# iric-soft/km

Hardware: AMD Instinct MI355X
Metric: find_mutation_targets_per_sec (higher is better)
Workload: dtype u64

## Files before the change

### km_amd/csrc/walk_kernel.h

```cpp
#pragma once
#include "device_common.h"

namespace kmd {

constexpr uint32_t ST_NODE = 1, ST_ONSTACK = 2, ST_POPPED = 3;
__device__ inline uint16_t slot_meta(uint32_t state, uint32_t idx) { return (uint16_t)((state << 14) | (idx & 0x3FFFu)); }
__device__ inline uint32_t meta_state(uint16_t m) { return (uint32_t)m >> 14; }
__device__ inline uint32_t meta_index(uint16_t m) { return (uint32_t)m & 0x3FFFu; }
constexpr uint32_t T_OK = 0, T_NODE_LIMIT = 1, T_REPEAT = 2, T_EMPTY = 3, T_BAD_BASE = 4,
                   T_INTERNAL = 5, T_NEEDS_BIG = 100;
constexpr uint64_t DFS_STEP_LIMIT = 1ull << 32;
constexpr uint32_t SEED_BLOCK = 256;

constexpr uint32_t POOL_GROUPS = 64;
constexpr uint32_t POOL_CTR_STRIDE = 16;
constexpr uint32_t NOT_BARE = 0xFFFFFFFFu;

struct EpiArgs {
  unsigned long long* counters;
  uint64_t path_pool, run_pool;
  uint32_t* p_target;
  uint64_t* p_runbase;
  uint32_t* p_nruns;
  uint32_t* p_len;
  uint32_t* p_mincov;
  uint32_t* r_start;
  uint32_t* r_len;
  uint32_t* g_status;
  uint32_t* t_npaths;
  uint32_t* t_pathbase;
  uint32_t* t_nruns;
  uint32_t* t_refmax;
  uint32_t* left;
  uint32_t* n_left;
  uint32_t* t_eremoved;
  uint32_t* t_enonref;
};
constexpr uint32_t EPI_CHUNKS = 3;
constexpr uint32_t EPI_MAX_BUBBLES = 8;

struct __attribute__((aligned(16))) BranchFrame {
  uint4 c4;
  uint32_t depth, mask, brk, pad;
};

struct WalkArgs {
  TableView tab;
  const uint8_t* bases;
  const uint64_t* toff;
  uint64_t* packed;
  const uint64_t* woff;
  uint32_t n_targets;
  double ratio;
  int64_t n_cutoff;
  double nc;
  uint64_t thr_below;
  uint32_t thr_T;
  uint32_t max_stack, max_break, max_node;
  uint64_t* items;
  const uint32_t* item_off;
  uint32_t n_items;
  uint32_t* flagbits;
  const uint64_t* fw_off;
  uint32_t* tflag;
  uint32_t* flagged;
  uint32_t* n_flagged;
  uint4* flag_rec;
  uint32_t fast_extra;
  const EpiArgs* epi;
  const uint32_t* list;
  const uint32_t* n_list_dev;
  uint32_t n_list_host;
  uint64_t* node_kmer;
  uint32_t* node_cnt;
  uint64_t* node_base;
  uint32_t* node_cap;
  const uint64_t* node_base0;
  uint32_t* big_ctl;
  uint32_t* big_walk;
  uint32_t big_slots;
  uint32_t big_entry;
  uint64_t big_region;
  uint32_t big_prep;
  uint32_t* loop_list;
  uint32_t* loop_ctl;
  uint32_t loop_cap;
  uint32_t* t_eremoved;
  uint32_t* t_enonref;
  uint32_t* n_nodes;
  uint32_t* n_ref;
  uint32_t* status;
  unsigned long long* probes;
  unsigned long long* dfs_probes;
  unsigned long long* fetches;
  uint32_t hs_cap;
  uint32_t pcap;
  uint32_t words_cap;
  uint32_t fcap;
  uint32_t bcap;
  uint32_t dbg;
  uint32_t spec;
  unsigned char* g_ws;
  uint64_t g_stride;
  unsigned char* f_ws;
  uint64_t f_stride;
  unsigned long long* stamps;
  unsigned long long* pool_counters;
};

__host__ __device__ inline uint64_t walk_frame_bytes(uint32_t fcap) {
  return (((uint64_t)fcap * 16) + 15) & ~15ull;
}
__host__ __device__ inline uint64_t walk_lds_bytes(uint32_t hs_cap, uint32_t words_cap, uint32_t bcap, uint32_t pcap,
                                                   uint32_t pos_elt) {
  uint64_t b = 0;
  b += (uint64_t)hs_cap * 8;
  b += (uint64_t)words_cap * 8;
  b += (uint64_t)bcap * 32;
  b += (uint64_t)hs_cap * 2;
  b += (uint64_t)pcap * pos_elt;
  return (b + 15) & ~15ull;
}
__host__ __device__ inline uint64_t walk_ws_bytes(uint32_t hs_cap, uint32_t words_cap,
                                                  uint32_t fcap, uint32_t bcap, uint32_t pcap) {
  return walk_lds_bytes(hs_cap, words_cap, bcap, pcap, 4) + walk_frame_bytes(fcap);
}

__device__ inline uint32_t set_home(uint64_t key, uint32_t cap) {
  uint32_t h = (uint32_t)key ^ ((uint32_t)(key >> 32) * 0x85EBCA6Bu);
  h *= 0x9E3779B1u;
  h ^= h >> 15;
  return __umulhi(h, cap);
}

template <int SH = 0>
__device__ inline int set_insert_lane(uint64_t* keys, uint32_t cap, uint64_t key, bool* was_new) {
  uint32_t s = set_home(key >> SH, cap);
  for (uint32_t step = 0; step < cap; ++step) {
    unsigned long long old = atomicCAS(reinterpret_cast<unsigned long long*>(&keys[s]),
                                       (unsigned long long)EMPTY, (unsigned long long)key);
    if (old == EMPTY) { *was_new = true; return (int)s; }
    if (old == key) { *was_new = false; return (int)s; }
    if (++s == cap) s = 0;
  }
  *was_new = false;
  return -1;
}

template <int SH = 0>
__device__ inline int set_lookup_lane(const uint64_t* keys, uint32_t cap, uint64_t key, bool* found) {
  uint32_t s = set_home(key >> SH, cap);
  for (uint32_t step = 0; step < cap; ++step) {
    const uint64_t kv = keys[s];
    if (kv == key) { *found = true; return (int)s; }
    if (kv == EMPTY) { *found = false; return (int)s; }
    if (++s == cap) s = 0;
  }
  *found = false;
  return -1;
}

template <int SH = 0>
__device__ inline int set_find(const uint64_t* keys, uint32_t cap, uint64_t key, bool* found) {
  const uint32_t lane = (uint32_t)lane_id();
  uint32_t base = set_home(key >> SH, cap);
  for (uint32_t scanned = 0; scanned < cap + 64; scanned += 64) {
    uint32_t s = base + lane;
    if (s >= cap) s -= cap;
    const uint64_t kv = keys[s];
    const unsigned long long mm = __ballot(kv == key);
    const unsigned long long me = __ballot(kv == EMPTY);
    if (mm | me) {
      const int lm = mm ? (__ffsll((long long)mm) - 1) : 64;
      const int le = me ? (__ffsll((long long)me) - 1) : 64;
      uint32_t pos = base + (uint32_t)(lm < le ? lm : le);
      if (pos >= cap) pos -= cap;
      *found = lm < le;
      return (int)pos;
    }
    base += 64;
    if (base >= cap) base -= cap;
  }
  *found = false;
  return -1;
}

constexpr uint32_t PACK_WAVES = 4;
__global__ __launch_bounds__(64 * PACK_WAVES) void k_pack(WalkArgs a) {
  constexpr uint32_t PACK_LDS_WORDS = 192;
  __shared__ uint64_t lds_words[PACK_WAVES][PACK_LDS_WORDS];
  uint64_t* const mine = lds_words[threadIdx.x >> 6];
  const uint32_t t = blockIdx.x * PACK_WAVES + (threadIdx.x >> 6);
  const uint32_t lane = (uint32_t)lane_id();
  if (t >= a.n_targets) return;
  const uint64_t off = a.toff[t];
  const uint64_t L = a.toff[t + 1] - off;
  const uint64_t wo = a.woff[t];
  const uint64_t fwo = a.fw_off[t];
  const uint64_t nbase = a.node_base0[t];
  const uint64_t item0 = a.item_off[t];
  const uint32_t nwords = (uint32_t)((L + 31) >> 5);
  const uint32_t n_ref = (L >= (uint64_t)a.tab.k) ? (uint32_t)(L - a.tab.k + 1) : 0;
  uint32_t bad = 0;
  for (uint32_t c = 0; c * 8 <= nwords; ++c) {
    const uint64_t p = (uint64_t)c * 256 + lane * 4;
    uint32_t byte = 0;
    uint32_t four = 0;
    if (p + 4 <= L) {
      __builtin_memcpy(&four, a.bases + off + p, 4);
    } else {
#pragma unroll
      for (uint32_t j = 0; j < 4; ++j)
        if (p + j < L) four |= (uint32_t)a.bases[off + p + j] << (8 * j);
    }
#pragma unroll
    for (uint32_t j = 0; j < 4; ++j) {
      uint32_t code = 0;
      if (p + j < L) {
        const uint32_t ch = (four >> (8 * j)) & 0xDFu;
        bad |= (ch != 'A' && ch != 'C' && ch != 'G' && ch != 'T') ? 1u : 0u;
        code = ((ch >> 1) ^ (ch >> 2)) & 3u;
      }
      byte = (byte << 2) | code;
    }
    uint64_t v = (uint64_t)byte << (56 - 8 * (lane & 7));
    v |= __shfl_xor(v, 1);
    v |= __shfl_xor(v, 2);
    v |= __shfl_xor(v, 4);
    const uint32_t w = c * 8 + (lane >> 3);
    if ((lane & 7) == 0 && w <= nwords) {
      a.packed[wo + w] = v;
      if (w < PACK_LDS_WORDS) mine[w] = v;
    }
  }
  const bool in_lds = nwords < PACK_LDS_WORDS;
  for (uint32_t w = lane; w < (n_ref + 31) / 32; w += 64) a.flagbits[fwo + w] = 0;
  const int any_bad = __any((int)bad);
  uint32_t st = T_OK;
  if (n_ref == 0) st = T_EMPTY;
  else if (any_bad) st = T_BAD_BASE;
  else if (a.max_stack > 0 && n_ref > a.max_node) st = T_NODE_LIMIT;
  if (in_lds) {
    asm volatile("s_waitcnt lgkmcnt(0)" ::: "memory");
  } else {
    __builtin_amdgcn_fence(__ATOMIC_RELEASE, "wavefront");
    asm volatile("s_waitcnt vmcnt(0)" ::: "memory");
    __builtin_amdgcn_fence(__ATOMIC_ACQUIRE, "wavefront");
  }
  {
    const uint32_t n_it = (n_ref + SEED_BLOCK - 1) / SEED_BLOCK;
    uint64_t* rec0 = a.items + 16ull * item0;
    for (uint32_t x = lane; x < n_it * 16; x += 64) {
      const uint32_t q = x >> 4, f = x & 15;
      uint64_t v;
      if (f == 0) v = (uint64_t)t | ((uint64_t)(q * SEED_BLOCK) << 32);
      else if (f == 1) v = (uint64_t)n_ref | ((uint64_t)(st == T_OK ? 1u : 0u) << 32);
      else if (f == 2) v = nbase;
      else if (f == 3) v = fwo | (wo << 32);
      else {
        const uint32_t w = q * (SEED_BLOCK / 32) + (f - 4);
        v = (w <= nwords) ? (in_lds ? mine[w] : a.packed[wo + w]) : 0ull;
      }
      rec0[x] = v;
    }
  }
  if (lane == 0) {
    a.status[t] = st;
    a.n_ref[t] = n_ref;
    a.n_nodes[t] = (st == T_OK || st == T_NODE_LIMIT) ? n_ref : 0;
    a.probes[t] = 0;
    a.dfs_probes[t] = 0;
    a.fetches[t] = 0;
    a.tflag[t] = 0;
    a.node_base[t] = nbase;
    a.node_cap[t] = n_ref + a.fast_extra;
    a.t_eremoved[t] = 0;
    a.t_enonref[t] = 0;
    if (t == 0) a.loop_ctl[0] = 0;
    if (t == 0 && a.big_ctl) { a.big_ctl[0] = 0; a.big_ctl[1] = 0; }
    if (t == 0) { a.n_flagged[0] = 0; a.n_flagged[1] = 0; a.n_flagged[2] = 0; }
  }
  {
    constexpr uint32_t CTR_PAIRS = (POOL_GROUPS * POOL_CTR_STRIDE + 16) / 2;
    ulonglong2* ctr = reinterpret_cast<ulonglong2*>(a.pool_counters);
    for (uint64_t i = (uint64_t)t * 64 + lane; i < CTR_PAIRS; i += (uint64_t)a.n_targets * 64)
      ctr[i] = make_ulonglong2(0ull, 0ull);
  }
}

#define KM_SEED_STAMP(n)                                                                  \
  do {                                                                                    \
    if constexpr (STAMPS) {                                                               \
      unsigned long long t_;                                                              \
      asm volatile("s_waitcnt vmcnt(0) lgkmcnt(0)\n\ts_memtime %0\n\ts_waitcnt lgkmcnt(0)" \
                   : "=s"(t_)::"memory");                                                 \
      ts[n] = t_;                                                                         \
    }                                                                                     \
  } while (0)

template <bool STAMPS, int K, bool FETCHES>
__global__ __launch_bounds__(SEED_BLOCK) void k_seed(WalkArgs a) {
  static_assert(SEED_BLOCK == 256, "the item record holds 12 words = 256 seeds + k - 1 + 1 bases");
  constexpr uint32_t RAW = SEED_BLOCK + 32;
  __shared__ uint32_t raw[RAW];
  unsigned long long ts[8] = {0, 0, 0, 0, 0, 0, 0, 0};
  unsigned long long real0 = 0;
  uint32_t probes_first = 0;
  if constexpr (STAMPS) real0 = __builtin_amdgcn_s_memrealtime();
  KM_SEED_STAMP(0);
  const TableView tab = specialized_view<K>(a.tab);
  const int k = tab.k;
  const uint32_t tid = threadIdx.x;
  const uint32_t lane = tid & 63u;
  const uint32_t W = (uint32_t)tab.w;
  const uint64_t* rec = a.items + 16ull * blockIdx.x;
  KM_SEED_STAMP(1);
  auto bits_at = [&](uint32_t q) -> uint64_t {
    const uint32_t w = q >> 5, sh = (q & 31) * 2;
    const uint64_t hi = rec[4 + w], lo = rec[5 + w];
    return (hi << sh) | ((lo >> 1) >> (63 - sh));
  };
  const uint64_t x = bits_at(tid);
  KM_SEED_STAMP(2);

  raw[tid] = mmer_scan_key(tab, x, tid);
  if (tid < W) raw[SEED_BLOCK + tid] = mmer_scan_key(tab, bits_at(SEED_BLOCK + tid), SEED_BLOCK + tid);
  const uint64_t h0 = rec[0], h1 = rec[1];
  const uint64_t nb = rec[2], fwo = rec[3] & 0xFFFFFFFFull;
  const uint32_t wo32 = (uint32_t)(rec[3] >> 32);
  if ((uint32_t)(h1 >> 32) == 0u) return;
  const uint32_t t = (uint32_t)h0;
  const uint32_t n_ref = (uint32_t)h1;
  const uint32_t i = (uint32_t)(h0 >> 32) + tid;
  __syncthreads();
  uint32_t m_rest;
  uint32_t m_last;
  if (W == 16) {
    const uint32_t* r = raw + tid + 1;
    const uint32_t m0 = min(min(r[0], r[1]), r[2]), m1 = min(min(r[3], r[4]), r[5]);
    const uint32_t m2 = min(min(r[6], r[7]), r[8]), m3 = min(min(r[9], r[10]), r[11]);
    const uint32_t m4 = min(min(r[12], r[13]), r[14]);
    m_rest = min(min(min(m0, m1), m2), min(m3, m4));
    m_last = r[15];
  } else {
    m_rest = ~0u;
    for (uint32_t j = 1; j < W; ++j) m_rest = min(m_rest, raw[tid + j]);
    m_last = raw[tid + W];
  }
  const uint32_t u_child = (min(m_rest, m_last) & SEL_POS) - (tid + 1);
  KM_SEED_STAMP(3);

  const uint64_t X = x >> (64 - 2 * k);
  const Key g = key_from_window(tab, X & tab.pmask, u_child);
  const DirPair dw = *reinterpret_cast<const DirPair*>(tab.dir + g.bucket);
  const bool head = i == 0;
  Key gq = g;
  DirPair dq = dw;
  if (head) {
    const uint32_t u_first = min(raw[0], m_rest) & SEL_POS;
    gq = key_from_window(tab, X >> 2, u_first);
    dq = *reinterpret_cast<const DirPair*>(tab.dir + gq.bucket);
  }
  KM_SEED_STAMP(4);
  const uint32_t S = (uint32_t)bucket_slots(dw.lo, dw.hi);
  const Slot* base = tab.slots + 2ull * dw.lo;
  const uint32_t pos = (uint32_t)home_slot(tab, g, S);
  const Slot* b0 = (S ? base : tab.slots) + pos;
  const uint4 first = *reinterpret_cast<const uint4*>(b0);
  const uint4 second = *reinterpret_cast<const uint4*>(b0 + 1);
  uint32_t Sq = 0, posq = 0;
  const Slot* baseq = tab.slots;
  uint4 firstq = first, secondq = second;
  if (head) {
    Sq = (uint32_t)bucket_slots(dq.lo, dq.hi);
    baseq = tab.slots + 2ull * dq.lo;
    posq = (uint32_t)home_slot(tab, gq, Sq);
    const Slot* bq = (Sq ? baseq : tab.slots) + posq;
    firstq = *reinterpret_cast<const uint4*>(bq);
    secondq = *reinterpret_cast<const uint4*>(bq + 1);
  }
  KM_SEED_STAMP(5);

  uint32_t fetch_l = 0;
  bool valid = false, triv = false, triv_child = false;
  if (i < n_ref) {
    valid = true;
    uint4 c4 = make_uint4(0, 0, 0, 0);
    if (S) c4 = bucket_resolve2(tab, g, base, S, pos, first, second, &fetch_l);
    c4 = finish_children(tab, X, g.flip, c4);
    KM_SEED_STAMP(6);
    if constexpr (STAMPS) probes_first = fetch_l;
    uint32_t nextb = 4;
    if (i + 1 < n_ref) {
      if (k < 32) {
        nextb = (uint32_t)(x >> (62 - 2 * k)) & 3u;
      } else {
        const uint32_t p = tid + (uint32_t)k;
        nextb = (uint32_t)(rec[4 + (p >> 5)] >> (62 - 2 * (p & 31))) & 3u;
      }
      a.node_cnt[nb + i + 1] = pick4(c4, nextb);
    }
    if (head) {
      uint4 cq = make_uint4(0, 0, 0, 0);
      if (Sq) cq = bucket_resolve2(tab, gq, baseq, Sq, posq, firstq, secondq, &fetch_l);
      const uint32_t sb = (uint32_t)(X & 3);
      uint32_t v = pick4(cq, gq.flip ? 3 - sb : sb);
      if (v == COUNT_ESCAPE) v = overflow_count(tab, X);
      a.node_cnt[nb] = v;
    }
    if (a.max_stack > 0) {
      const uint32_t mask = child_mask(c4, a.ratio, a.nc);
      triv = (mask == 0) || (nextb < 4 && mask == (1u << nextb));
      triv_child = triv && mask != 0;
      if (!triv) {
        atomicOr(&a.flagbits[fwo + (i >> 5)], 1u << (i & 31));
        if (atomicExch(&a.tflag[t], 1u) == 0u) {
          const uint32_t at = atomicAdd(a.n_flagged, 1u);
          a.flagged[at] = t;
          a.flag_rec[2 * at] = make_uint4(t, n_ref, (uint32_t)nb, (uint32_t)(nb >> 32));
          a.flag_rec[2 * at + 1] = make_uint4((uint32_t)fwo, wo32, 0u, 0u);
        }
      }
    }
  }
  const unsigned long long probes_w = (unsigned long long)__popcll(__ballot(valid)) +
                                      4ull * __popcll(__ballot(triv)) + __popcll(__ballot(triv_child));
  unsigned long long fetch_w = 0;
  if constexpr (FETCHES || STAMPS) {
    fetch_w = (unsigned long long)__popcll(__ballot(fetch_l >= 1)) + __popcll(__ballot(fetch_l >= 2));
    if (__any(fetch_l > 2)) {
      uint32_t extra = fetch_l > 2 ? fetch_l - 2 : 0;
      for (int o = 32; o > 0; o >>= 1) extra += __shfl_xor(extra, o);
      fetch_w += extra;
    }
  }
  if (lane == 0 && probes_w) {
    atomicAdd(&a.probes[t], probes_w);
    if constexpr (FETCHES || STAMPS) atomicAdd(&a.fetches[t], fetch_w);
  }
  if constexpr (STAMPS) {
    KM_SEED_STAMP(7);
    const unsigned long long real1 = __builtin_amdgcn_s_memrealtime();
    uint32_t pmax = probes_first, psum = probes_first;
    for (int o2 = 32; o2 > 0; o2 >>= 1) {
      const uint32_t v = __shfl_xor(pmax, o2);
      pmax = v > pmax ? v : pmax;
      psum += __shfl_xor(psum, o2);
    }
    if (lane == 0) {
      unsigned long long* o = a.stamps + 16ull * (blockIdx.x * (SEED_BLOCK / 64) + (tid >> 6));
      for (int q = 0; q < 8; ++q) o[q] = ts[q];
      o[8] = real0; o[9] = real1;
      o[10] = __builtin_amdgcn_s_getreg((31 << 11) | 4);
      o[11] = __builtin_amdgcn_s_getreg((31 << 11) | 20);
      o[12] = pmax; o[13] = psum;
    }
  }
}

constexpr uint32_t SEED_WAVE_KEYS = 96;
constexpr int SEED_WAVE_RUNS = 4;
constexpr uint32_t SEED_WAVE_LDS = SEED_WAVE_RUNS * SEED_WAVE_KEYS * 4;
template <int K, bool FETCHES, int NS>
__device__ __forceinline__ void seed_body(const WalkArgs a, const uint32_t item, const uint32_t wave) {
  static_assert(SEED_BLOCK == 256, "the item record holds 12 words = 256 seeds + k - 1 + 1 bases");
  static_assert(NS == 1 || NS == 2 || NS == 4, "one, two or all four runs of 64 seeds per wave");
  constexpr uint32_t WAVES = 4 / NS;
  extern __shared__ __align__(16) unsigned char smem[];
  uint32_t* const raw_all = reinterpret_cast<uint32_t*>(smem);
  const TableView tab = specialized_view<K>(a.tab);
  const int k = tab.k;
  const uint32_t lane = (uint32_t)lane_id();
  const uint32_t W = (uint32_t)tab.w;
  const uint64_t* rec = a.items + 16ull * item;
  auto bits_at = [&](uint32_t q) -> uint64_t {
    const uint32_t w = q >> 5, sh = (q & 31) * 2;
    const uint64_t hi = rec[4 + w], lo = rec[5 + w];
    return (hi << sh) | ((lo >> 1) >> (63 - sh));
  };
  struct Run {
    uint32_t tid, m_rest, u_child, S, pos;
    uint64_t x, X;
    Key g;
    DirPair dw;
    const Slot* base;
    uint4 first, second;
  };
  Run r0, r1, r2, r3;
  auto hash_keys = [&](Run& r, const uint32_t j) {
    r.tid = 64u * (wave + WAVES * j) + lane;
    r.x = bits_at(r.tid);
    uint32_t* raw = raw_all + SEED_WAVE_KEYS * j;
    raw[lane] = mmer_scan_key(tab, r.x, r.tid);
    if (lane < W) raw[64 + lane] = mmer_scan_key(tab, bits_at(r.tid + 64), r.tid + 64);
  };
  hash_keys(r0, 0);
  if constexpr (NS >= 2) hash_keys(r1, 1);
  if constexpr (NS == 4) { hash_keys(r2, 2); hash_keys(r3, 3); }
  const uint64_t h0 = rec[0], h1 = rec[1];
  const uint64_t nb = rec[2], fwo = rec[3] & 0xFFFFFFFFull;
  const uint32_t wo32 = (uint32_t)(rec[3] >> 32);
  if ((uint32_t)(h1 >> 32) == 0u) return;
  const uint32_t t = (uint32_t)h0;
  const uint32_t n_ref = (uint32_t)h1;
  const uint32_t i_first = (uint32_t)(h0 >> 32);
  if (i_first + 64u * wave >= n_ref) return;
  asm volatile("s_waitcnt lgkmcnt(0)" ::: "memory");
  auto minimizer = [&](Run& r, const uint32_t j) {
    const uint32_t* w = raw_all + SEED_WAVE_KEYS * j + lane + 1;
    uint32_t m_last;
    if (W == 16) {
      const uint32_t m0 = min(min(w[0], w[1]), w[2]), m1 = min(min(w[3], w[4]), w[5]);
      const uint32_t m2 = min(min(w[6], w[7]), w[8]), m3 = min(min(w[9], w[10]), w[11]);
      const uint32_t m4 = min(min(w[12], w[13]), w[14]);
      r.m_rest = min(min(min(m0, m1), m2), min(m3, m4));
      m_last = w[15];
    } else {
      r.m_rest = ~0u;
      for (uint32_t q = 1; q < W; ++q) r.m_rest = min(r.m_rest, w[q - 1]);
      m_last = w[W - 1];
    }
    r.u_child = (min(r.m_rest, m_last) & SEL_POS) - (r.tid + 1);
  };
  minimizer(r0, 0);
  if constexpr (NS >= 2) minimizer(r1, 1);
  if constexpr (NS == 4) { minimizer(r2, 2); minimizer(r3, 3); }

  auto directory = [&](Run& r) {
    r.X = r.x >> (64 - 2 * k);
    r.g = key_from_window(tab, r.X & tab.pmask, r.u_child);
    r.dw = *reinterpret_cast<const DirPair*>(tab.dir + r.g.bucket);
  };
  directory(r0);
  if constexpr (NS >= 2) directory(r1);
  if constexpr (NS == 4) { directory(r2); directory(r3); }
  const bool head = i_first + r0.tid == 0;
  Key gq = r0.g;
  DirPair dq = r0.dw;
  if (head) {
    const uint32_t u_first = min(raw_all[0], r0.m_rest) & SEL_POS;
    gq = key_from_window(tab, r0.X >> 2, u_first);
    dq = *reinterpret_cast<const DirPair*>(tab.dir + gq.bucket);
  }
  auto home_pair = [&](Run& r) {
    r.S = (uint32_t)bucket_slots(r.dw.lo, r.dw.hi);
    r.base = tab.slots + 2ull * r.dw.lo;
    r.pos = (uint32_t)home_slot(tab, r.g, r.S);
    const Slot* b0 = (r.S ? r.base : tab.slots) + r.pos;
    r.first = *reinterpret_cast<const uint4*>(b0);
    r.second = *reinterpret_cast<const uint4*>(b0 + 1);
  };
  home_pair(r0);
  if constexpr (NS >= 2) home_pair(r1);
  if constexpr (NS == 4) { home_pair(r2); home_pair(r3); }
  uint32_t Sq = 0, posq = 0;
  const Slot* baseq = tab.slots;
  uint4 firstq = r0.first, secondq = r0.second;
  if (head) {
    Sq = (uint32_t)bucket_slots(dq.lo, dq.hi);
    baseq = tab.slots + 2ull * dq.lo;
    posq = (uint32_t)home_slot(tab, gq, Sq);
    const Slot* bq = (Sq ? baseq : tab.slots) + posq;
    firstq = *reinterpret_cast<const uint4*>(bq);
    secondq = *reinterpret_cast<const uint4*>(bq + 1);
  }

  unsigned long long probes_w = 0, fetch_w = 0;
  auto classify = [&](Run& r, const bool with_head) {
    const uint32_t i = i_first + r.tid;
    uint32_t fetch_l = 0;
    bool valid = false, triv = false, triv_child = false;
    if (i < n_ref) {
      valid = true;
      uint4 c4 = make_uint4(0, 0, 0, 0);
      if (r.S) c4 = bucket_resolve2(tab, r.g, r.base, r.S, r.pos, r.first, r.second, &fetch_l);
      c4 = finish_children(tab, r.X, r.g.flip, c4);
      uint32_t nextb = 4;
      if (i + 1 < n_ref) {
        if (k < 32) {
          nextb = (uint32_t)(r.x >> (62 - 2 * k)) & 3u;
        } else {
          const uint32_t p = r.tid + (uint32_t)k;
          nextb = (uint32_t)(rec[4 + (p >> 5)] >> (62 - 2 * (p & 31))) & 3u;
        }
        a.node_cnt[nb + i + 1] = pick4(c4, nextb);
      }
      if (with_head && head) {
        uint4 cq = make_uint4(0, 0, 0, 0);
        if (Sq) cq = bucket_resolve2(tab, gq, baseq, Sq, posq, firstq, secondq, &fetch_l);
// ... 1019 lines not shown
```

Before: 64.74 million.

## Rework pack kernel with 16-byte chunk loads and register-resident item records

Rewrites k_pack so each lane loads 16-byte aligned chunks of bases, encodes them with SWAR bit tricks, and assembles 64-bit packed words via shuffles. For short targets the item records are filled from registers instead of reading the packed buffer back, and per-target header fields are loaded by separate lanes and broadcast with readlane. Per-target status stores are gathered through LDS into one coalesced write per block, and the block grows to 8 waves. This adds code complexity and a block-wide barrier in exchange for fewer, wider memory transactions.

```diff
diff --git a/km_amd/csrc/pack_map.h b/km_amd/csrc/pack_map.h
--- /dev/null
+++ b/km_amd/csrc/pack_map.h
@@ -0,0 +1,77 @@
+#pragma once
+#include <stdint.h>
+
+#if defined(__HIPCC__) || defined(__CUDACC__)
+#define KM_PACK_HD __host__ __device__
+#else
+#define KM_PACK_HD
+#endif
+
+enum : uint32_t {
+  PACK_CHUNK_BASES = 16,
+  PACK_TRIP_CHUNKS = 64,
+  PACK_TRIP_BASES = PACK_CHUNK_BASES * PACK_TRIP_CHUNKS,
+  PACK_TRIP_WORDS = PACK_TRIP_BASES / 32,
+  PACK_ZERO_LANE = 1,
+  PACK_ITEM_SEEDS = 256,
+  PACK_ITEM_FIELDS = 16,
+  PACK_ITEM_HEADER = 4,
+  PACK_NONE = 0xFFFFFFFFu,
+};
+
+KM_PACK_HD inline uint32_t pack_misalign(uint64_t address) { return (uint32_t)(address & (PACK_CHUNK_BASES - 1)); }
+KM_PACK_HD inline uint32_t pack_nwords(uint64_t L) { return (uint32_t)((L + 31) >> 5); }
+KM_PACK_HD inline uint32_t pack_trips(uint64_t L) { return (uint32_t)((L + PACK_TRIP_BASES - 1) / PACK_TRIP_BASES); }
+
+struct PackRange { uint64_t lo, hi; };
+KM_PACK_HD inline PackRange pack_chunk_bases(uint64_t j, uint32_t m, uint64_t L) {
+  const uint64_t end = PACK_CHUNK_BASES * j + PACK_CHUNK_BASES - m;
+  const uint64_t lo = end > PACK_CHUNK_BASES ? end - PACK_CHUNK_BASES : 0;
+  const uint64_t hi = end < L ? end : L;
+  return PackRange{lo, hi > lo ? hi : lo};
+}
+KM_PACK_HD inline bool pack_chunks_from(uint64_t j, uint32_t m, uint64_t L) {
+  return j == 0 ? L > 0 : PACK_CHUNK_BASES * j - m < L;
+}
+KM_PACK_HD inline uint32_t pack_chunk_trip(uint64_t j) { return (uint32_t)(j / PACK_TRIP_CHUNKS); }
+KM_PACK_HD inline uint32_t pack_chunk_lane(uint64_t j) { return (uint32_t)(j % PACK_TRIP_CHUNKS); }
+KM_PACK_HD inline uint32_t pack_word_trip(uint32_t w) { return w / PACK_TRIP_WORDS; }
+KM_PACK_HD inline uint32_t pack_word_lane(uint32_t w) { return 2 * (w % PACK_TRIP_WORDS); }
+
+KM_PACK_HD inline uint32_t pack_codes4(uint32_t four) {
+  const uint32_t x = four & 0xDFDFDFDFu;
+  const uint32_t c = ((x >> 1) ^ (x >> 2)) & 0x03030303u;
+  return (c * 0x40100401u) >> 24;
+}
+KM_PACK_HD inline uint32_t pack_bad4(uint32_t four) {
+  const uint32_t x = four & 0xDFDFDFDFu;
+  const uint32_t c = (x >> 1) ^ (x >> 2);
+  const uint32_t b0 = c & 0x01010101u, b1 = (c >> 1) & 0x01010101u;
+  const uint32_t t = b0 & b1;
+  const uint32_t want = 0x40404040u | ((b0 ^ b1) << 1) | (b1 << 2) | (t << 4) | (t ^ 0x01010101u);
+  return want ^ x;
+}
+KM_PACK_HD inline uint32_t pack_codes16(uint32_t d0, uint32_t d1, uint32_t d2, uint32_t d3) {
+  return (pack_codes4(d0) << 24) | (pack_codes4(d1) << 16) | (pack_codes4(d2) << 8) | pack_codes4(d3);
+}
+KM_PACK_HD inline uint32_t pack_half(uint32_t own, uint32_t next, uint32_t m) {
+  return m ? (own << (2 * m)) | (next >> (32 - 2 * m)) : own;
+}
+
+KM_PACK_HD inline uint32_t pack_item_word(uint32_t q, uint32_t f) { return q * (PACK_ITEM_SEEDS / 32) + (f - PACK_ITEM_HEADER); }
+KM_PACK_HD inline uint32_t pack_n_items(uint32_t n_ref) { return (n_ref + PACK_ITEM_SEEDS - 1) / PACK_ITEM_SEEDS; }
+KM_PACK_HD inline bool pack_items_from_registers(uint64_t L, uint32_t n_ref) {
+  return L <= PACK_TRIP_BASES && pack_n_items(n_ref) * PACK_ITEM_FIELDS <= 64;
+}
+KM_PACK_HD inline uint32_t pack_item_source_lane(uint32_t lane, uint32_t nwords) {
+  const uint32_t q = lane / PACK_ITEM_FIELDS, f = lane % PACK_ITEM_FIELDS;
+  if (f < PACK_ITEM_HEADER) return PACK_NONE;
+  const uint32_t w = pack_item_word(q, f);
+  return w < nwords ? pack_word_lane(w) : PACK_NONE;
+}
+
+KM_PACK_HD inline uint32_t pack_scalar_target(uint32_t block, uint32_t wave, uint32_t lane, uint32_t waves, uint32_t n_targets) {
+  if (wave != 0 || lane >= waves) return PACK_NONE;
+  const uint64_t t = (uint64_t)block * waves + lane;
+  return t < n_targets ? (uint32_t)t : PACK_NONE;
+}
diff --git a/km_amd/csrc/walk_kernel.h b/km_amd/csrc/walk_kernel.h
--- a/km_amd/csrc/walk_kernel.h
+++ b/km_amd/csrc/walk_kernel.h
@@ -1,5 +1,6 @@
 #pragma once
 #include "device_common.h"
+#include "pack_map.h"
 
 namespace kmd {
 
@@ -185,106 +186,149 @@
   return -1;
 }
 
-constexpr uint32_t PACK_WAVES = 4;
+constexpr uint32_t PACK_WAVES = 8;
+static_assert(SEED_BLOCK == PACK_ITEM_SEEDS, "pack_map.h has the item record's geometry");
+
+__device__ inline uint32_t pack_chunk(uint64_t base0, uint32_t m, uint64_t L, uint64_t j, uint32_t& bad) {
+  const PackRange r = pack_chunk_bases(j, m, L);
+  uint32_t d0 = 0x41414141u, d1 = d0, d2 = d0, d3 = d0;
+  const uint64_t chunk = base0 + PACK_CHUNK_BASES * j - m;
+  if (r.hi - r.lo == PACK_CHUNK_BASES) {
+    const uint4 v = *reinterpret_cast<const uint4*>(chunk);
+    d0 = v.x; d1 = v.y; d2 = v.z; d3 = v.w;
+  } else if (r.hi > r.lo) {
+    const uint8_t* p = reinterpret_cast<const uint8_t*>(chunk);
+    const uint32_t lo = (uint32_t)(base0 + r.lo - chunk), hi = (uint32_t)(base0 + r.hi - chunk);
+    uint32_t ch[PACK_CHUNK_BASES];
+#pragma unroll
+    for (uint32_t i = 0; i < PACK_CHUNK_BASES; ++i) ch[i] = p[i < lo ? lo : (i >= hi ? hi - 1 : i)];
+    uint32_t d[4] = {0, 0, 0, 0};
+#pragma unroll
+    for (uint32_t i = 0; i < PACK_CHUNK_BASES; ++i) {
+      const uint32_t in = (uint32_t)-(int32_t)(i >= lo && i < hi);
+      d[i >> 2] |= ((ch[i] & in) | (0x41u & ~in)) << (8 * (i & 3));
+    }
+    d0 = d[0]; d1 = d[1]; d2 = d[2]; d3 = d[3];
+  }
+  bad |= pack_bad4(d0) | pack_bad4(d1) | pack_bad4(d2) | pack_bad4(d3);
+  return pack_codes16(d0, d1, d2, d3);
+}
+
+__device__ inline uint64_t pack_lane64(uint64_t v, int src) {
+  const uint32_t lo = (uint32_t)__builtin_amdgcn_readlane((int)(uint32_t)v, src);
+  const uint32_t hi = (uint32_t)__builtin_amdgcn_readlane((int)(uint32_t)(v >> 32), src);
+  return ((uint64_t)hi << 32) | lo;
+}
+
 __global__ __launch_bounds__(64 * PACK_WAVES) void k_pack(WalkArgs a) {
-  constexpr uint32_t PACK_LDS_WORDS = 192;
-  __shared__ uint64_t lds_words[PACK_WAVES][PACK_LDS_WORDS];
-  uint64_t* const mine = lds_words[threadIdx.x >> 6];
-  const uint32_t t = blockIdx.x * PACK_WAVES + (threadIdx.x >> 6);
+  __shared__ uint32_t wave_status[PACK_WAVES];
+  const uint32_t wave = (uint32_t)__builtin_amdgcn_readfirstlane((int)(threadIdx.x >> 6));
   const uint32_t lane = (uint32_t)lane_id();
-  if (t >= a.n_targets) return;
-  const uint64_t off = a.toff[t];
-  const uint64_t L = a.toff[t + 1] - off;
-  const uint64_t wo = a.woff[t];
-  const uint64_t fwo = a.fw_off[t];
-  const uint64_t nbase = a.node_base0[t];
-  const uint64_t item0 = a.item_off[t];
-  const uint32_t nwords = (uint32_t)((L + 31) >> 5);
+  const uint32_t t = blockIdx.x * PACK_WAVES + wave;
+  const uint32_t ts = pack_scalar_target(blockIdx.x, wave, lane, PACK_WAVES, a.n_targets);
+  uint64_t s_off = 0, s_end = 0, s_nbase = 0;
+  if (ts != PACK_NONE) { s_off = a.toff[ts]; s_end = a.toff[ts + 1]; s_nbase = a.node_base0[ts]; }
+  if (t < a.n_targets) {
+  const uint64_t* hp = lane == 0 ? a.toff + t : lane == 1 ? a.toff + t + 1 : lane == 2 ? a.woff + t
+                     : lane == 3 ? a.fw_off + t : a.node_base0 + t;
+  const uint64_t hv = *hp;
+  const uint32_t iv = a.item_off[t];
+  const uint64_t off = pack_lane64(hv, 0);
+  const uint64_t L = pack_lane64(hv, 1) - off;
+  const uint64_t wo = pack_lane64(hv, 2);
+  const uint64_t fwo = pack_lane64(hv, 3);
+  const uint64_t nbase = pack_lane64(hv, 4);
+  const uint64_t item0 = (uint32_t)__builtin_amdgcn_readfirstlane((int)iv);
+  {
+    constexpr uint32_t CTR_PAIRS = (POOL_GROUPS * POOL_CTR_STRIDE + 16) / 2;
+    ulonglong2* ctr = reinterpret_cast<ulonglong2*>(a.pool_counters);
+    for (uint64_t i = (uint64_t)t * 64 + lane; i < CTR_PAIRS; i += (uint64_t)a.n_targets * 64)
+      ctr[i] = make_ulonglong2(0ull, 0ull);
+  }
+  const uint32_t nwords = pack_nwords(L);
   const uint32_t n_ref = (L >= (uint64_t)a.tab.k) ? (uint32_t)(L - a.tab.k + 1) : 0;
+  for (uint32_t w = lane; w < (n_ref + 31) / 32; w += 64) a.flagbits[fwo + w] = 0;
+  if (lane == PACK_ZERO_LANE) a.packed[wo + nwords] = 0ull;
+  if (lane == 0 && t == 0) {
+    a.loop_ctl[0] = 0;
+    if (a.big_ctl) { a.big_ctl[0] = 0; a.big_ctl[1] = 0; }
+    a.n_flagged[0] = 0; a.n_flagged[1] = 0; a.n_flagged[2] = 0;
+  }
+  const uint64_t base0 = reinterpret_cast<uint64_t>(a.bases) + off;
+  const uint32_t m = pack_misalign(base0);
+  const uint32_t trips = pack_trips(L);
   uint32_t bad = 0;
-  for (uint32_t c = 0; c * 8 <= nwords; ++c) {
-    const uint64_t p = (uint64_t)c * 256 + lane * 4;
-    uint32_t byte = 0;
-    uint32_t four = 0;
-    if (p + 4 <= L) {
-      __builtin_memcpy(&four, a.bases + off + p, 4);
-    } else {
-#pragma unroll
-      for (uint32_t j = 0; j < 4; ++j)
-        if (p + j < L) four |= (uint32_t)a.bases[off + p + j] << (8 * j);
-    }
-#pragma unroll
-    for (uint32_t j = 0; j < 4; ++j) {
-      uint32_t code = 0;
-      if (p + j < L) {
-        const uint32_t ch = (four >> (8 * j)) & 0xDFu;
-        bad |= (ch != 'A' && ch != 'C' && ch != 'G' && ch != 'T') ? 1u : 0u;
-        code = ((ch >> 1) ^ (ch >> 2)) & 3u;
-      }
-      byte = (byte << 2) | code;
-    }
-    uint64_t v = (uint64_t)byte << (56 - 8 * (lane & 7));
-    v |= __shfl_xor(v, 1);
-    v |= __shfl_xor(v, 2);
-    v |= __shfl_xor(v, 4);
-    const uint32_t w = c * 8 + (lane >> 3);
-    if ((lane & 7) == 0 && w <= nwords) {
-      a.packed[wo + w] = v;
-      if (w < PACK_LDS_WORDS) mine[w] = v;
-    }
-  }
-  const bool in_lds = nwords < PACK_LDS_WORDS;
-  for (uint32_t w = lane; w < (n_ref + 31) / 32; w += 64) a.flagbits[fwo + w] = 0;
+  uint64_t v = 0;
+  uint32_t own = pack_chunks_from(0, m, L) ? pack_chunk(base0, m, L, lane, bad) : 0u;
+  for (uint32_t c = 0; c < trips; ++c) {
+    const uint64_t j1 = (uint64_t)(c + 1) * PACK_TRIP_CHUNKS;
+    const uint32_t ahead = pack_chunks_from(j1, m, L) ? pack_chunk(base0, m, L, j1 + lane, bad) : 0u;
+    uint32_t next = __shfl_down(own, 1);
+    const uint32_t first_ahead = __shfl(ahead, 0);
+    if (lane == PACK_TRIP_CHUNKS - 1) next = first_ahead;
+    const uint32_t half = pack_half(own, next, m);
+    const uint32_t mate = __shfl_xor(half, 1);
+    v = (lane & 1) ? (((uint64_t)mate << 32) | half) : (((uint64_t)half << 32) | mate);
+    const uint32_t w = c * PACK_TRIP_WORDS + (lane >> 1);
+    if ((lane & 1) == 0 && w < nwords) a.packed[wo + w] = v;
+    own = ahead;
+  }
   const int any_bad = __any((int)bad);
   uint32_t st = T_OK;
   if (n_ref == 0) st = T_EMPTY;
   else if (any_bad) st = T_BAD_BASE;
   else if (a.max_stack > 0 && n_ref > a.max_node) st = T_NODE_LIMIT;
-  if (in_lds) {
-    asm volatile("s_waitcnt lgkmcnt(0)" ::: "memory");
+  if (lane == 0) wave_status[wave] = st;
+  const uint32_t n_it = pack_n_items(n_ref);
+  uint64_t* rec0 = a.items + 16ull * item0;
+  const uint64_t head1 = (uint64_t)n_ref | ((uint64_t)(st == T_OK ? 1u : 0u) << 32);
+  const uint64_t head3 = fwo | (wo << 32);
+  if (pack_items_from_registers(L, n_ref)) {
+    const uint32_t q = lane / PACK_ITEM_FIELDS, f = lane % PACK_ITEM_FIELDS;
+    const uint32_t src = pack_item_source_lane(lane, nwords);
+    const uint64_t word = __shfl(v, (int)(src == PACK_NONE ? 0u : src));
+    uint64_t x;
+    if (f == 0) x = (uint64_t)t | ((uint64_t)(q * SEED_BLOCK) << 32);
+    else if (f == 1) x = head1;
+    else if (f == 2) x = nbase;
+    else if (f == 3) x = head3;
+    else x = src == PACK_NONE ? 0ull : word;
+    if (lane < n_it * PACK_ITEM_FIELDS) rec0[lane] = x;
   } else {
     __builtin_amdgcn_fence(__ATOMIC_RELEASE, "wavefront");
     asm volatile("s_waitcnt vmcnt(0)" ::: "memory");
     __builtin_amdgcn_fence(__ATOMIC_ACQUIRE, "wavefront");
-  }
-  {
-    const uint32_t n_it = (n_ref + SEED_BLOCK - 1) / SEED_BLOCK;
-    uint64_t* rec0 = a.items + 16ull * item0;
-    for (uint32_t x = lane; x < n_it * 16; x += 64) {
-      const uint32_t q = x >> 4, f = x & 15;
-      uint64_t v;
-      if (f == 0) v = (uint64_t)t | ((uint64_t)(q * SEED_BLOCK) << 32);
-      else if (f == 1) v = (uint64_t)n_ref | ((uint64_t)(st == T_OK ? 1u : 0u) << 32);
-      else if (f == 2) v = nbase;
-      else if (f == 3) v = fwo | (wo << 32);
+    for (uint32_t i = lane; i < n_it * PACK_ITEM_FIELDS; i += 64) {
+      const uint32_t q = i / PACK_ITEM_FIELDS, f = i % PACK_ITEM_FIELDS;
+      uint64_t x;
+      if (f == 0) x = (uint64_t)t | ((uint64_t)(q * SEED_BLOCK) << 32);
+      else if (f == 1) x = head1;
+      else if (f == 2) x = nbase;
+      else if (f == 3) x = head3;
       else {
-        const uint32_t w = q * (SEED_BLOCK / 32) + (f - 4);
-        v = (w <= nwords) ? (in_lds ? mine[w] : a.packed[wo + w]) : 0ull;
-      }
-      rec0[x] = v;
-    }
-  }
-  if (lane == 0) {
-    a.status[t] = st;
-    a.n_ref[t] = n_ref;
-    a.n_nodes[t] = (st == T_OK || st == T_NODE_LIMIT) ? n_ref : 0;
-    a.probes[t] = 0;
-    a.dfs_probes[t] = 0;
-    a.fetches[t] = 0;
-    a.tflag[t] = 0;
-    a.node_base[t] = nbase;
-    a.node_cap[t] = n_ref + a.fast_extra;
-    a.t_eremoved[t] = 0;
-    a.t_enonref[t] = 0;
-    if (t == 0) a.loop_ctl[0] = 0;
-    if (t == 0 && a.big_ctl) { a.big_ctl[0] = 0; a.big_ctl[1] = 0; }
-    if (t == 0) { a.n_flagged[0] = 0; a.n_flagged[1] = 0; a.n_flagged[2] = 0; }
-  }
-  {
-    constexpr uint32_t CTR_PAIRS = (POOL_GROUPS * POOL_CTR_STRIDE + 16) / 2;
-    ulonglong2* ctr = reinterpret_cast<ulonglong2*>(a.pool_counters);
-    for (uint64_t i = (uint64_t)t * 64 + lane; i < CTR_PAIRS; i += (uint64_t)a.n_targets * 64)
-      ctr[i] = make_ulonglong2(0ull, 0ull);
+        const uint32_t w = pack_item_word(q, f);
+        x = (w < nwords) ? a.packed[wo + w] : 0ull;
+      }
+      rec0[i] = x;
+    }
+  }
+  }
+  __syncthreads();
+  if (ts != PACK_NONE) {
+    const uint32_t st = wave_status[lane];
+    const uint64_t L = s_end - s_off;
+    const uint32_t n_ref = (L >= (uint64_t)a.tab.k) ? (uint32_t)(L - a.tab.k + 1) : 0;
+    a.status[ts] = st;
+    a.n_ref[ts] = n_ref;
+    a.n_nodes[ts] = (st == T_OK || st == T_NODE_LIMIT) ? n_ref : 0;
+    a.probes[ts] = 0;
+    a.dfs_probes[ts] = 0;
+    a.fetches[ts] = 0;
+    a.tflag[ts] = 0;
+    a.node_base[ts] = s_nbase;
+    a.node_cap[ts] = n_ref + a.fast_extra;
+    a.t_eremoved[ts] = 0;
+    a.t_enonref[ts] = 0;
   }
 }
 
```

Measured after the change: 65.11 million (median of 4 runs). About the same (+0.6%).
